# aniketntnu/WordDiffusion

Hardware: AMD Instinct MI355X
Metric: denoised 64x256 word images/sec (1000-step DDPM), whole job (higher is better)
Workload: dtype bf16x3; 1 GPU; BASELINE configs[1]: batch 64 per GPU of 64x256 crops = [64,4,8,32] latents, 1000-step DDPM (999 executed steps), base unet.py UNetModel (320 ch, mult (1,1), 4 heads, 339 writers), random-init synthetic weights; variant=base, batch_per_gpu=64, noise_steps=1000, executed_steps_per_image=999, precision=split-bf16 MFMA x3, fp32 accumulate (<=1e-4 of the fp32 reference), output_finite=True

## Files before the change

worddiffusion_amd/csrc/wd_ff.hip:

```cpp
#include "wd_gemm_epi.h"

namespace {

constexpr int FNT = 512;
constexpr int FBM = 64;
constexpr int FC = 320;
constexpr int FCH = 128;
constexpr int FRING = 6;
constexpr int F_MAX_INNER = 2048;
constexpr int FGRP = 30;
constexpr uint32_t F_OOB = 0x80000000u;

typedef __attribute__((ext_vector_type(4))) unsigned f_u32x4;

__device__ __forceinline__ int f_lds_off(int row, int ch) { return row * 128 + ((ch ^ ((row >> 1) & 7)) << 4); }

template <int NPASS, bool PROJ, bool FRONT>
__global__ void __launch_bounds__(FNT, 1) wd_ff_kernel(const wd_ff_args a) {
#if defined(__HIP_DEVICE_COMPILE__)
    static_assert(!FRONT || (NPASS == 3 && PROJ), "the transformer front needs split-bf16 operands and the proj_out tail");
    constexpr int NPL = (NPASS == 1) ? 1 : 2;
    constexpr int SLAB = 2 * FBM * 128;
    constexpr int A_BYTES = 5 * SLAB;
    constexpr int H_BYTES = 2 * SLAB;
    extern __shared__ __attribute__((aligned(16))) char smem[];
    char* s_a = smem;
    char* s_h = smem + A_BYTES;
    float* s_b1 = reinterpret_cast<float*>(smem + A_BYTES + 2 * H_BYTES);

    const int m0 = blockIdx.x * FBM;
    const int tid = threadIdx.x;
    const int lane = tid & 63;
    const int wave = __builtin_amdgcn_readfirstlane(tid >> 6);
    const int kh = wave >> 2, cg = wave & 3;
    const int l15 = lane & 15, lq = lane >> 4;
    const int nchunk = a.inner / FCH;

    auto make_srd = [](const wd_bf16* p) {
        return __builtin_amdgcn_make_buffer_rsrc(const_cast<wd_bf16*>(p), 0, 0x7FFFFFF0, 0x00020000);
    };
    const __amdgpu_buffer_rsrc_t srd1_hi = make_srd(a.w1_hi), srd1_lo = make_srd(a.w1_lo ? a.w1_lo : a.w1_hi);
    const __amdgpu_buffer_rsrc_t srd2_hi = make_srd(a.w2_hi), srd2_lo = make_srd(a.w2_lo ? a.w2_lo : a.w2_hi);
    const __amdgpu_buffer_rsrc_t srd3_hi = make_srd(PROJ ? a.w3_hi : a.w2_hi), srd3_lo = make_srd(PROJ ? (a.w3_lo ? a.w3_lo : a.w3_hi) : a.w2_hi);
    const uint32_t lane16 = lane * 16;
    const int nct1 = (2 * a.inner) >> 4;

    bf16x8 ring[FRING][NPL];
    auto issue = [&](const int slot, const int g, const int j) {
        const bool live = j < nchunk;
        const uint32_t vo = live ? lane16 : F_OOB;
        if (PROJ && g < FRING) {
            const uint32_t so3 = (uint32_t)(((2 * (g / 5) + kh) * (FC / 16) + 5 * cg + g % 5) * 1024);
            const uint32_t so1 = (uint32_t)(((g >> 1) * nct1 + 2 * (j * 8 + wave) + (g & 1)) * 1024);
            const uint32_t so = live ? so1 : so3;
#pragma unroll
            for (int p = 0; p < NPL; ++p) {
                const __amdgpu_buffer_rsrc_t srd = live ? (p ? srd1_lo : srd1_hi) : (p ? srd3_lo : srd3_hi);
                ring[slot][p] = __builtin_bit_cast(bf16x8, __builtin_amdgcn_raw_buffer_load_b128(srd, lane16, so, 0));
            }
        } else if (g < 20) {
            const uint32_t so = (uint32_t)(((g >> 1) * nct1 + 2 * (j * 8 + wave) + (g & 1)) * 1024);
#pragma unroll
            for (int p = 0; p < NPL; ++p)
                ring[slot][p] = __builtin_bit_cast(bf16x8, __builtin_amdgcn_raw_buffer_load_b128(p ? srd1_lo : srd1_hi, vo, live ? so : 0u, 0));
        } else {
            const int q = (g - 20) / 5, t = (g - 20) % 5;
            const uint32_t so = (uint32_t)(((4 * j + 2 * kh + q) * (FC / 16) + 5 * cg + t) * 1024);
#pragma unroll
            for (int p = 0; p < NPL; ++p)
                ring[slot][p] = __builtin_bit_cast(bf16x8, __builtin_amdgcn_raw_buffer_load_b128(p ? srd2_lo : srd2_hi, vo, live ? so : 0u, 0));
        }
    };
    f32x4 acc2[4][5];
    bf16x8 xa[4][NPL];
    auto read_frags = [&](const char* slab_base, const int half) {
        const int ch = half * 4 + lq;
#pragma unroll
        for (int i = 0; i < 4; ++i) {
            const int ao = f_lds_off(i * 16 + l15, ch);
#pragma unroll
            for (int p = 0; p < NPL; ++p) xa[i][p] = *reinterpret_cast<const bf16x8*>(slab_base + p * (FBM * 128) + ao);
        }
    };
    auto mfma12 = [&](f32x4 (&acc)[4], const bf16x8 (&w)[NPL]) {
#pragma unroll
        for (int i = 0; i < 4; ++i) {
            if (NPL == 2) {
                acc[i] = __builtin_amdgcn_mfma_f32_16x16x32_bf16(xa[i][NPL - 1], w[0], acc[i], 0, 0, 0);
                acc[i] = __builtin_amdgcn_mfma_f32_16x16x32_bf16(xa[i][0], w[NPL - 1], acc[i], 0, 0, 0);
            }
            acc[i] = __builtin_amdgcn_mfma_f32_16x16x32_bf16(xa[i][0], w[0], acc[i], 0, 0, 0);
        }
    };
    constexpr int LDE = FC + 4;
    float* ep = reinterpret_cast<float*>(smem);
    auto ksum_to_image = [&]() {
        for (int hh = 0; hh < 2; ++hh) {
            if (kh == hh) {
#pragma unroll
                for (int i = 0; i < 4; ++i)
#pragma unroll
                    for (int t = 0; t < 5; ++t)
#pragma unroll
                        for (int r = 0; r < 4; ++r) {
                            float* pe = ep + (i * 16 + 4 * lq + r) * LDE + cg * 80 + t * 16 + l15;
                            *pe = (hh == 0) ? acc2[i][t][r] : *pe + acc2[i][t][r];
                        }
            }
            __syncthreads();
        }
    };

    if constexpr (FRONT) {
        constexpr int SP = 65, PP = 72, KS32 = FC / 32;
        const int b = m0 / a.hw;
        const int HJ = a.heads * a.L;
        char* fr = s_h + 4096;
        float* s_aff = reinterpret_cast<float*>(fr);
        float* sS = reinterpret_cast<float*>(fr);
        wd_bf16* sP = reinterpret_cast<wd_bf16*>(fr + FBM * SP * 4);
        {
            const int ngp = FC / a.gn_pcpg, ratio = a.gn_cpg / a.gn_pcpg;
            for (int c = tid; c < FC; c += FNT) {
                const int g = c / a.gn_cpg;
                double su = 0.0, sq = 0.0;
                for (int k = 0; k < ratio; ++k)
                    for (int ck = 0; ck < a.gn_nchunk; ++ck) {
                        const double* pp = a.gn_part + (((long)b * a.gn_nchunk + ck) * ngp + g * ratio + k) * 2;
                        su += pp[0];
                        sq += pp[1];
                    }
                const double n = (double)a.hw * a.gn_cpg;
                const double mu = su / n;
                double var = sq / n - mu * mu;
                if (var < 0.0) var = 0.0;
                const float rstd = (float)(1.0 / sqrt(var + (double)a.gn_eps));
                const float sc = rstd * a.gn_gamma[c];
                s_aff[2 * c] = sc;
                s_aff[2 * c + 1] = a.gn_beta[c] - (float)mu * sc;
            }
            for (int e = tid; e < FBM * PP; e += FNT) reinterpret_cast<uint32_t*>(sP)[e] = 0u;
        }
        const int arow = tid >> 3, ach = tid & 7;
        float4 xv[5][2];
        {
            const float* xrow = a.x_in + (long)(m0 + arow) * a.x_in_ld + ach * 8;
#pragma unroll
            for (int sl = 0; sl < 5; ++sl) {
                xv[sl][0] = *reinterpret_cast<const float4*>(xrow + sl * 64);
                xv[sl][1] = *reinterpret_cast<const float4*>(xrow + sl * 64 + 4);
            }
        }
        const __amdgpu_buffer_rsrc_t srdp_hi = make_srd(a.pi_hi), srdp_lo = make_srd(a.pi_lo);
        auto issue_pi = [&](const int slot, const int g) {
            const uint32_t so = (uint32_t)(((2 * (g / 5) + kh) * (FC / 16) + 5 * cg + g % 5) * 1024);
#pragma unroll
            for (int p = 0; p < NPL; ++p)
                ring[slot][p] = __builtin_bit_cast(bf16x8, __builtin_amdgcn_raw_buffer_load_b128(p ? srdp_lo : srdp_hi, lane16, so, 0));
        };
#pragma unroll
        for (int g = 0; g < FRING; ++g) issue_pi(g, g);
        __syncthreads();
#pragma unroll
        for (int sl = 0; sl < 5; ++sl) {
            const float4* tab = reinterpret_cast<const float4*>(s_aff + 2 * (sl * 64 + ach * 8));
            const float4 t0 = tab[0], t1 = tab[1], t2 = tab[2], t3 = tab[3];
            const float4 x0 = xv[sl][0], x1 = xv[sl][1];
            float4 y0, y1;
            y0.x = x0.x * t0.x + t0.y; y0.y = x0.y * t0.z + t0.w; y0.z = x0.z * t1.x + t1.y; y0.w = x0.w * t1.z + t1.w;
            y1.x = x1.x * t2.x + t2.y; y1.y = x1.y * t2.z + t2.w; y1.z = x1.z * t3.x + t3.y; y1.w = x1.w * t3.z + t3.w;
            uint2 h0, l0, h1, l1;
            wd_split4(y0, h0, l0);
            wd_split4(y1, h1, l1);
            char* dst = s_a + sl * SLAB + f_lds_off(arow, ach);
            *reinterpret_cast<f_u32x4*>(dst) = f_u32x4{h0.x, h0.y, h1.x, h1.y};
            *reinterpret_cast<f_u32x4*>(dst + FBM * 128) = f_u32x4{l0.x, l0.y, l1.x, l1.y};
        }
        __syncthreads();
#pragma unroll
        for (int i = 0; i < 4; ++i)
#pragma unroll
            for (int t = 0; t < 5; ++t)
#pragma unroll
                for (int r = 0; r < 4; ++r) acc2[i][t][r] = 0.0f;
#pragma unroll
        for (int g = 0; g < 25; ++g) {
            const int q = g / 5, t = g % 5;
            if (t == 0) read_frags(s_a + q * SLAB, kh);
            {
                f32x4 col[4] = {acc2[0][t], acc2[1][t], acc2[2][t], acc2[3][t]};
                mfma12(col, ring[g % FRING]);
#pragma unroll
                for (int i = 0; i < 4; ++i) acc2[i][t] = col[i];
            }
            if (g + FRING < 25) issue_pi(g % FRING, g + FRING);
            __builtin_amdgcn_sched_barrier(0);
        }
        __syncthreads();
        ksum_to_image();
        float4 xr[2][5];
#pragma unroll
        for (int pp = 0; pp < 2; ++pp)
#pragma unroll
            for (int i = 0; i < 5; ++i) {
                const int n = (l15 + 16 * i) * 4, row = wave * 8 + pp * 4 + lq;
                const float4 v = *reinterpret_cast<const float4*>(ep + row * LDE + n);
                const float4 bx = *reinterpret_cast<const float4*>(a.pi_b + n);
                xr[pp][i] = make_float4(v.x + bx.x, v.y + bx.y, v.z + bx.z, v.w + bx.w);
            }
        __syncthreads();
        auto ln_rows = [&](const float* gamma, const float* beta) {
#pragma unroll
            for (int pp = 0; pp < 2; ++pp) {
                const int row = wave * 8 + pp * 4 + lq;
                float s = 0.f;
#pragma unroll
                for (int i = 0; i < 5; ++i) s += (xr[pp][i].x + xr[pp][i].y) + (xr[pp][i].z + xr[pp][i].w);
                const float mean = wd_row16_sum(s) / (float)FC;
                float q = 0.f;
#pragma unroll
                for (int i = 0; i < 5; ++i) {
                    const float a0 = xr[pp][i].x - mean, a1 = xr[pp][i].y - mean, a2 = xr[pp][i].z - mean, a3 = xr[pp][i].w - mean;
                    q += (a0 * a0 + a1 * a1) + (a2 * a2 + a3 * a3);
                }
                const float rstd = 1.0f / sqrtf(wd_row16_sum(q) / (float)FC + a.ln_eps);
#pragma unroll
                for (int i = 0; i < 5; ++i) {
                    const int n = (l15 + 16 * i) * 4;
                    const float4 ga = *reinterpret_cast<const float4*>(gamma + n);
                    const float4 be = *reinterpret_cast<const float4*>(beta + n);
                    const float4 x = xr[pp][i];
                    float4 o;
                    o.x = (x.x - mean) * rstd * ga.x + be.x; o.y = (x.y - mean) * rstd * ga.y + be.y;
                    o.z = (x.z - mean) * rstd * ga.z + be.z; o.w = (x.w - mean) * rstd * ga.w + be.w;
                    uint2 hi, lo;
                    wd_split4(o, hi, lo);
                    char* d = s_a + (n >> 6) * SLAB + f_lds_off(row, (n & 63) >> 3) + (n & 7) * 2;
                    *reinterpret_cast<uint2*>(d) = hi;
                    *reinterpret_cast<uint2*>(d + FBM * 128) = lo;
                }
            }
        };
        const int ht = wave & 3, rp = wave >> 2;
        const long pq = 64L * FC;
#pragma unroll
        for (int ps = 0; ps < 2; ++ps) {
            const wd_bf16* mq = ps == 0 ? a.mq_a : a.mq_b;
            const wd_bf16* mot = ps == 0 ? a.mot_a : a.mot_b;
            const float* xb = ps == 0 ? a.xb_a : a.xb_b;
            ln_rows(a.ln2_gamma, a.ln2_beta);
            __builtin_amdgcn_sched_barrier(0);
            bf16x8 bh[KS32], bl[KS32];
            {
                const __amdgpu_buffer_rsrc_t rq = __builtin_amdgcn_make_buffer_rsrc(const_cast<wd_bf16*>(mq + (long)b * 2 * pq), 0,
                                                                                    (int)(2 * pq * 2), 0x00020000);
                const uint32_t vo = ht * 16 + l15 < HJ ? lane16 : F_OOB;
#pragma unroll
                for (int ks = 0; ks < KS32; ++ks) {
                    bh[ks] = __builtin_bit_cast(bf16x8, __builtin_amdgcn_raw_buffer_load_b128(rq, vo, (uint32_t)((ht * KS32 + ks) << 10), 0));
                    bl[ks] = __builtin_bit_cast(bf16x8, __builtin_amdgcn_raw_buffer_load_b128(rq, vo, (uint32_t)(((ht * KS32 + ks) << 10) + pq * 2), 0));
                }
            }
            __syncthreads();
            if (ht * 16 < HJ) {
                f32x4 a_lh[2], a_hl[2], a_hh[2];
#pragma unroll
                for (int ri = 0; ri < 2; ++ri)
#pragma unroll
                    for (int r = 0; r < 4; ++r) a_lh[ri][r] = a_hl[ri][r] = a_hh[ri][r] = 0.f;
#pragma unroll
                for (int ks = 0; ks < KS32; ++ks)
#pragma unroll
                    for (int ri = 0; ri < 2; ++ri) {
                        const char* ap = s_a + (ks >> 1) * SLAB + f_lds_off((2 * rp + ri) * 16 + l15, (ks & 1) * 4 + lq);
                        const bf16x8 ah = *reinterpret_cast<const bf16x8*>(ap);
                        const bf16x8 al = *reinterpret_cast<const bf16x8*>(ap + FBM * 128);
                        a_lh[ri] = __builtin_amdgcn_mfma_f32_16x16x32_bf16(al, bh[ks], a_lh[ri], 0, 0, 0);
                        a_hl[ri] = __builtin_amdgcn_mfma_f32_16x16x32_bf16(ah, bl[ks], a_hl[ri], 0, 0, 0);
                        a_hh[ri] = __builtin_amdgcn_mfma_f32_16x16x32_bf16(ah, bh[ks], a_hh[ri], 0, 0, 0);
                    }
#pragma unroll
                for (int ri = 0; ri < 2; ++ri)
#pragma unroll
                    for (int r = 0; r < 4; ++r)
                        sS[((2 * rp + ri) * 16 + 4 * lq + r) * SP + ht * 16 + l15] = (a_lh[ri][r] + a_hl[ri][r]) + a_hh[ri][r];
            }
            __builtin_amdgcn_sched_barrier(0);
            bf16x8 mh[2][5], ml[2][5];
            {
                const __amdgpu_buffer_rsrc_t rm = __builtin_amdgcn_make_buffer_rsrc(const_cast<wd_bf16*>(mot + (long)b * 2 * pq), 0,
                                                                                    (int)(2 * pq * 2), 0x00020000);
#pragma unroll
                for (int ks = 0; ks < 2; ++ks) {
                    const uint32_t vo = ks * 32 + lq * 8 < HJ ? lane16 : F_OOB;
#pragma unroll
                    for (int t = 0; t < 5; ++t) {
                        const uint32_t so = (uint32_t)((((5 * cg + t) * 2 + ks) << 10));
                        mh[ks][t] = __builtin_bit_cast(bf16x8, __builtin_amdgcn_raw_buffer_load_b128(rm, vo, so, 0));
                        ml[ks][t] = __builtin_bit_cast(bf16x8, __builtin_amdgcn_raw_buffer_load_b128(rm, vo, so + (uint32_t)(pq * 2), 0));
                    }
                }
            }
            __syncthreads();
            for (int idx = tid; idx < FBM * a.heads; idx += FNT) {
                const int t = idx / a.heads, h = idx - t * a.heads;
                const float* pr = sS + t * SP + h * a.L;
                wd_bf16* ph = sP + t * PP + h * a.L;
                float mx = -3.4e38f;
                for (int j = 0; j < a.L; ++j) mx = fmaxf(mx, pr[j]);
                float sum = 0.f;
                for (int j = 0; j < a.L; ++j) sum += __expf(pr[j] - mx);
                const float inv = __fdividef(1.f, sum);
                for (int j = 0; j < a.L; ++j) {
                    uint32_t hi, lo;
                    wd_split1(__expf(pr[j] - mx) * inv, hi, lo);
                    ph[j] = (wd_bf16)hi;
                    ph[FBM * PP + j] = (wd_bf16)lo;
                }
            }
            __syncthreads();
            {
                f32x4 o[2][5];
#pragma unroll
                for (int ri = 0; ri < 2; ++ri)
#pragma unroll
                    for (int t = 0; t < 5; ++t)
#pragma unroll
                        for (int r = 0; r < 4; ++r) o[ri][t][r] = 0.f;
#pragma unroll
                for (int ks = 0; ks < 2; ++ks)
#pragma unroll
                    for (int ri = 0; ri < 2; ++ri) {
                        const wd_bf16* ap = sP + ((2 * rp + ri) * 16 + l15) * PP + lq * 8 + ks * 32;
                        const bf16x8 ah = *reinterpret_cast<const bf16x8*>(ap);
                        const bf16x8 al = *reinterpret_cast<const bf16x8*>(ap + FBM * PP);
#pragma unroll
                        for (int t = 0; t < 5; ++t) o[ri][t] = __builtin_amdgcn_mfma_f32_16x16x32_bf16(al, mh[ks][t], o[ri][t], 0, 0, 0);
#pragma unroll
                        for (int t = 0; t < 5; ++t) o[ri][t] = __builtin_amdgcn_mfma_f32_16x16x32_bf16(ah, ml[ks][t], o[ri][t], 0, 0, 0);
#pragma unroll
                        for (int t = 0; t < 5; ++t) o[ri][t] = __builtin_amdgcn_mfma_f32_16x16x32_bf16(ah, mh[ks][t], o[ri][t], 0, 0, 0);
                    }
#pragma unroll
                for (int ri = 0; ri < 2; ++ri)
#pragma unroll
                    for (int t = 0; t < 5; ++t)
#pragma unroll
                        for (int r = 0; r < 4; ++r) ep[((2 * rp + ri) * 16 + 4 * lq + r) * LDE + (5 * cg + t) * 16 + l15] = o[ri][t][r];
            }
            __syncthreads();
#pragma unroll
            for (int pp = 0; pp < 2; ++pp)
#pragma unroll
                for (int i = 0; i < 5; ++i) {
                    const int n = (l15 + 16 * i) * 4, row = wave * 8 + pp * 4 + lq;
                    const float4 bi = *reinterpret_cast<const float4*>(xb + n);
                    const float4 at = *reinterpret_cast<const float4*>(ep + row * LDE + n);
                    const float4 x = xr[pp][i];
                    xr[pp][i] = make_float4(at.x + bi.x + x.x, at.y + bi.y + x.y, at.z + bi.z + x.z, at.w + bi.w + x.w);
                }
            __syncthreads();
        }
#pragma unroll
        for (int pp = 0; pp < 2; ++pp)
#pragma unroll
            for (int i = 0; i < 5; ++i)
                *reinterpret_cast<float4*>(a.tok2 + (long)(m0 + wave * 8 + pp * 4 + lq) * FC + (l15 + 16 * i) * 4) = xr[pp][i];
        ln_rows(a.ln3_gamma, a.ln3_beta);
        for (int i = tid; i < 2 * a.inner; i += FNT) s_b1[i] = a.b1 ? a.b1[i] : 0.0f;
        __builtin_amdgcn_sched_barrier(0);
#pragma unroll
        for (int g = 0; g < FRING; ++g) issue(g, g, 0);
    } else {
#pragma unroll
    for (int g = 0; g < FRING; ++g) issue(g, g, 0);

    {
        const __amdgpu_buffer_rsrc_t sx_hi = make_srd(a.x_hi), sx_lo = make_srd(a.x_lo ? a.x_lo : a.x_hi);
        const int arow = tid >> 3, ach = tid & 7;
        const uint32_t vo = (m0 + arow < a.m) ? (uint32_t)(m0 + arow) * (uint32_t)(a.x_ld * 2) + (uint32_t)(ach * 16) : F_OOB;
        f_u32x4 v[5][NPL];
#pragma unroll
        for (int sl = 0; sl < 5; ++sl)
#pragma unroll
            for (int p = 0; p < NPL; ++p) v[sl][p] = __builtin_amdgcn_raw_buffer_load_b128(p ? sx_lo : sx_hi, vo, sl * 128, 0);
        const int dst = f_lds_off(arow, ach);
#pragma unroll
        for (int sl = 0; sl < 5; ++sl)
#pragma unroll
            for (int p = 0; p < NPL; ++p) *reinterpret_cast<f_u32x4*>(s_a + sl * SLAB + p * (FBM * 128) + dst) = v[sl][p];
        for (int i = tid; i < 2 * a.inner; i += FNT) s_b1[i] = a.b1 ? a.b1[i] : 0.0f;
    }
    }
    __syncthreads();

#pragma unroll
    for (int i = 0; i < 4; ++i)
#pragma unroll
        for (int t = 0; t < 5; ++t)
#pragma unroll
            for (int r = 0; r < 4; ++r) acc2[i][t][r] = 0.0f;

    for (int j = 0; j < nchunk; ++j) {
        char* hbuf = s_h + (j & 1) * H_BYTES;
        f32x4 ax[4], ag[4];
#pragma unroll
        for (int i = 0; i < 4; ++i)
#pragma unroll
            for (int r = 0; r < 4; ++r) {
                ax[i][r] = 0.0f;
                ag[i][r] = 0.0f;
            }
#pragma unroll
        for (int g = 0; g < 20; ++g) {
            if ((g & 1) == 0) read_frags(s_a + (g >> 2) * SLAB, (g >> 1) & 1);
            if (g & 1) mfma12(ag, ring[g % FRING]);
            else mfma12(ax, ring[g % FRING]);
            if (g + FRING < FGRP) issue(g % FRING, g + FRING, j);
            else issue(g % FRING, g + FRING - FGRP, j + 1);
            __builtin_amdgcn_sched_barrier(0);
        }
        {
            const int hcol = (j * 8 + wave) * 32 + l15;
            const float bx = s_b1[hcol], bg = s_b1[hcol + 16];
            const int slab = wave >> 2, ch = (wave & 3) * 2 + (l15 >> 3), e = (l15 & 7) * 2;
#pragma unroll
            for (int i = 0; i < 4; ++i)
#pragma unroll
                for (int r = 0; r < 4; ++r) {
                    const float h = (ax[i][r] + bx) * wd_gelu_erf(ag[i][r] + bg);
                    uint32_t hb, lb;
                    wd_split1(h, hb, lb);
                    char* p = hbuf + slab * SLAB + f_lds_off(i * 16 + lq * 4 + r, ch) + e;
                    *reinterpret_cast<unsigned short*>(p) = (unsigned short)hb;
                    if (NPL == 2) *reinterpret_cast<unsigned short*>(p + FBM * 128) = (unsigned short)lb;
                }
        }
        __syncthreads();
#pragma unroll
        for (int g = 20; g < FGRP; ++g) {
            const int q = (g - 20) / 5, t = (g - 20) % 5;
            if (t == 0) read_frags(hbuf + kh * SLAB, q);
            {
                f32x4 col[4] = {acc2[0][t], acc2[1][t], acc2[2][t], acc2[3][t]};
                mfma12(col, ring[g % FRING]);
#pragma unroll
                for (int i = 0; i < 4; ++i) acc2[i][t] = col[i];
            }
            if (g + FRING < FGRP) issue(g % FRING, g + FRING, j);
            else issue(g % FRING, g + FRING - FGRP, j + 1);
            __builtin_amdgcn_sched_barrier(0);
        }
    }

    __syncthreads();
    ksum_to_image();
    wd_gemm_args e = {};
    e.m = a.m;
    e.n = FC;
    e.hw_out = a.hw_out > 0 ? a.hw_out : 1;
    e.act = WD_ACT_NONE;
    e.out_f32 = a.out_f32;
    e.out_ld = a.out_ld;
    e.out_hi = a.out_hi;
    e.out_lo = a.out_lo;
    e.out_pl_ld = a.out_pl_ld;
    e.ksplit = 1;
    e.stat_part = a.stat_part;
    e.stat_cpg = a.stat_cpg;
    if constexpr (!PROJ) {
        e.bias = a.b2;
        e.resid = a.resid;
        e.resid_ld = a.resid_ld;
        wd_epilogue_from_image<FBM, FC, FNT>(e, ep, m0, 0, tid);
    } else {
        constexpr int ROWB = LDE * 4;
        const float* resid = FRONT ? a.tok2 : a.resid;
        const int resid_ld = FRONT ? FC : a.resid_ld;
        if (FRONT) asm volatile("s_waitcnt vmcnt(0)" ::: "memory");
        {
            float4 v[10];
#pragma unroll
            for (int it = 0; it < 10; ++it) {
                const int idx = it * 64 + lane, row = wave * 8 + idx / 80, c = (idx % 80) * 4;
                const int m = m0 + row;
                float4 x = *reinterpret_cast<const float4*>(ep + row * LDE + c);
                if (a.b2) {
                    const float4 q = *reinterpret_cast<const float4*>(a.b2 + c);
                    x.x += q.x; x.y += q.y; x.z += q.z; x.w += q.w;
                }
                if (resid && m < a.m) {
                    const float4 q = *reinterpret_cast<const float4*>(resid + (long)m * resid_ld + c);
                    x.x += q.x; x.y += q.y; x.z += q.z; x.w += q.w;
                }
                v[it] = x;
            }
            asm volatile("s_waitcnt lgkmcnt(0)" ::: "memory");
            __builtin_amdgcn_sched_barrier(0);
#pragma unroll
            for (int it = 0; it < 10; ++it) {
                const int idx = it * 64 + lane, row = wave * 8 + idx / 80, c = (idx % 80) * 4;
                uint2 hh, ll;
                wd_split4(v[it], hh, ll);
                char* rowp = reinterpret_cast<char*>(ep) + row * ROWB;
                *reinterpret_cast<uint2*>(rowp + c * 2) = hh;
                if (NPL == 2) *reinterpret_cast<uint2*>(rowp + 640 + c * 2) = ll;
            }
        }
        __syncthreads();
#pragma unroll
        for (int i = 0; i < 4; ++i)
#pragma unroll
            for (int t = 0; t < 5; ++t)
#pragma unroll
                for (int r = 0; r < 4; ++r) acc2[i][t][r] = 0.0f;
#pragma unroll
        for (int g = 0; g < 25; ++g) {
            const int q = g / 5, t = g % 5;
            if (t == 0) {
                const int ks = 2 * q + kh;
#pragma unroll
                for (int i = 0; i < 4; ++i) {
                    const char* rp = reinterpret_cast<const char*>(ep) + (i * 16 + l15) * ROWB + (ks * 4 + lq) * 16;
#pragma unroll
                    for (int p = 0; p < NPL; ++p) xa[i][p] = *reinterpret_cast<const bf16x8*>(rp + p * 640);
// ... 85 lines not shown
```

worddiffusion_amd/csrc/wd_norm.hip:

```cpp
#include "wd_common.h"

namespace {

constexpr int GN_TOK = 32;

__global__ void gn_stats_kernel(const float* __restrict__ x, int ld, int hw, int c, int cpg, int nchunk,
                                double* __restrict__ part) {
    extern __shared__ __attribute__((aligned(16))) char smem[];
    float* s_sum = reinterpret_cast<float*>(smem);
    float* s_sq = s_sum + 2 * c;
    const int b = blockIdx.y, j = blockIdx.x;
    const int cx = threadIdx.x * 4;
    const int t0 = j * GN_TOK, t1 = min(hw, t0 + GN_TOK);
    if (cx < c) {
        float4 s = make_float4(0, 0, 0, 0), q = make_float4(0, 0, 0, 0);
        const float* base = x + ((long)b * hw) * ld + cx;
        for (int t = t0 + threadIdx.y; t < t1; t += 2) {
            const float4 v = *reinterpret_cast<const float4*>(base + (long)t * ld);
            s.x += v.x; s.y += v.y; s.z += v.z; s.w += v.w;
            q.x += v.x * v.x; q.y += v.y * v.y; q.z += v.z * v.z; q.w += v.w * v.w;
        }
        *reinterpret_cast<float4*>(s_sum + threadIdx.y * c + cx) = s;
        *reinterpret_cast<float4*>(s_sq + threadIdx.y * c + cx) = q;
    }
// ... 51 lines not shown
    }
    __syncthreads();
    const int c4 = c >> 2;
    const int t0 = blockIdx.x * AP_TOK, nt = min(AP_TOK, hw - t0);
    if (c4 <= 256) {
        const int rpp = 256 / c4;
        const int tl = threadIdx.x / c4, cx = (threadIdx.x - tl * c4) * 4;
        if (tl >= rpp) return;
        float sc[4], sh[4];
#pragma unroll
        for (int j = 0; j < 4; ++j) {
            const int g = (cx + j) / cpg;
            sc[j] = s_rstd[g] * gamma[c_off + cx + j];
            sh[j] = beta[c_off + cx + j] - s_mean[g] * sc[j];
        }
        for (int t = tl; t < nt; t += rpp) {
            const long row = (long)b * hw + t0 + t;
            const long srow = sr.perm ? (long)b * hw + sr.perm[t0 + t] : row;
            const float4 v = *reinterpret_cast<const float4*>(x + srow * ld + cx);
            float4 y = make_float4(v.x * sc[0] + sh[0], v.y * sc[1] + sh[1], v.z * sc[2] + sh[2], v.w * sc[3] + sh[3]);
            if (silu) {
                y.x = wd_silu(y.x); y.y = wd_silu(y.y); y.z = wd_silu(y.z); y.w = wd_silu(y.w);
            }
            uint2 h, l;
            wd_split4(y, h, l);
            const long o = row * out_ld + c_off + cx;
            *reinterpret_cast<uint2*>(out_hi + o) = h;
            if (out_lo) *reinterpret_cast<uint2*>(out_lo + o) = l;
            if (raw_hi) {
                wd_split4(v, h, l);
                *reinterpret_cast<uint2*>(raw_hi + o) = h;
                if (raw_lo) *reinterpret_cast<uint2*>(raw_lo + o) = l;
            }
        }
        return;
    }
    const int total = nt * c4;
    for (int i = threadIdx.x; i < total; i += blockDim.x) {
        const int t = i / c4, cx = (i - t * c4) * 4;
        const long row = (long)b * hw + t0 + t;
        const long srow = sr.perm ? (long)b * hw + sr.perm[t0 + t] : row;
        const float4 v = *reinterpret_cast<const float4*>(x + srow * ld + cx);
        float4 y;
        {
            const int g = cx / cpg, g1 = (cx + 1) / cpg, g2 = (cx + 2) / cpg, g3 = (cx + 3) / cpg;
            const float4 ga = *reinterpret_cast<const float4*>(gamma + c_off + cx);
            const float4 be = *reinterpret_cast<const float4*>(beta + c_off + cx);
            const float s0 = s_rstd[g] * ga.x, s1 = s_rstd[g1] * ga.y, s2 = s_rstd[g2] * ga.z, s3 = s_rstd[g3] * ga.w;
            y.x = v.x * s0 + (be.x - s_mean[g] * s0);
            y.y = v.y * s1 + (be.y - s_mean[g1] * s1);
            y.z = v.z * s2 + (be.z - s_mean[g2] * s2);
            y.w = v.w * s3 + (be.w - s_mean[g3] * s3);
        }
        if (silu) {
            y.x = wd_silu(y.x); y.y = wd_silu(y.y); y.z = wd_silu(y.z); y.w = wd_silu(y.w);
        }
        uint2 h, l;
        wd_split4(y, h, l);
        const long o = row * out_ld + c_off + cx;
        *reinterpret_cast<uint2*>(out_hi + o) = h;
        if (out_lo) *reinterpret_cast<uint2*>(out_lo + o) = l;
        if (raw_hi) {
            wd_split4(v, h, l);
            *reinterpret_cast<uint2*>(raw_hi + o) = h;
            if (raw_lo) *reinterpret_cast<uint2*>(raw_lo + o) = l;
        }
    }
}

constexpr int LN_MAX4 = 8;
__global__ void layernorm_kernel(const float* __restrict__ x, int ld, int rows, int c, const float* __restrict__ gamma,
                                 const float* __restrict__ beta, float eps, wd_bf16* __restrict__ out_hi,
                                 wd_bf16* __restrict__ out_lo, int out_ld) {
    const int lane = threadIdx.x & 63;
    const int row = blockIdx.x * (blockDim.x >> 6) + (threadIdx.x >> 6);
    if (row >= rows) return;
    const int c4 = c >> 2;
    float4 v[LN_MAX4];
    float s = 0.f;
#pragma unroll
    for (int i = 0; i < LN_MAX4; ++i) {
        const int f = lane + 64 * i;
        if (f < c4) {
            v[i] = *reinterpret_cast<const float4*>(x + (long)row * ld + f * 4);
            s += (v[i].x + v[i].y) + (v[i].z + v[i].w);
        }
    }
    const float mean = wd_wave_sum(s) / (float)c;
    float q = 0.f;
#pragma unroll
    for (int i = 0; i < LN_MAX4; ++i) {
        const int f = lane + 64 * i;
        if (f < c4) {
            const float a = v[i].x - mean, b = v[i].y - mean, cc = v[i].z - mean, d = v[i].w - mean;
            q += (a * a + b * b) + (cc * cc + d * d);
        }
    }
    const float rstd = 1.0f / sqrtf(wd_wave_sum(q) / (float)c + eps);
#pragma unroll
    for (int i = 0; i < LN_MAX4; ++i) {
        const int f = lane + 64 * i;
        if (f < c4) {
            const float4 ga = *reinterpret_cast<const float4*>(gamma + f * 4);
            const float4 be = *reinterpret_cast<const float4*>(beta + f * 4);
            float4 y;
            y.x = (v[i].x - mean) * rstd * ga.x + be.x;
            y.y = (v[i].y - mean) * rstd * ga.y + be.y;
            y.z = (v[i].z - mean) * rstd * ga.z + be.z;
            y.w = (v[i].w - mean) * rstd * ga.w + be.w;
            uint2 h, l;
            wd_split4(y, h, l);
            const long o = (long)row * out_ld + f * 4;
            *reinterpret_cast<uint2*>(out_hi + o) = h;
            if (out_lo) *reinterpret_cast<uint2*>(out_lo + o) = l;
        }
    }
}

__global__ void split_kernel(const float* __restrict__ x, int ld, int rows, int c, int silu,
                             wd_bf16* __restrict__ out_hi, wd_bf16* __restrict__ out_lo, int out_ld) {
    const int c4 = c >> 2;
    const long total = (long)rows * c4;
    for (long i = (long)blockIdx.x * blockDim.x + threadIdx.x; i < total; i += (long)gridDim.x * blockDim.x) {
        const long r = i / c4;
        const int cx = (int)(i - r * c4) * 4;
        float4 v = *reinterpret_cast<const float4*>(x + r * ld + cx);
        if (silu) {
            v.x = wd_silu(v.x); v.y = wd_silu(v.y); v.z = wd_silu(v.z); v.w = wd_silu(v.w);
        }
        uint2 h, l;
        wd_split4(v, h, l);
        *reinterpret_cast<uint2*>(out_hi + r * out_ld + cx) = h;
        if (out_lo) *reinterpret_cast<uint2*>(out_lo + r * out_ld + cx) = l;
    }
}

constexpr int GC_CH = 64;
constexpr int GC_PITCH = GC_CH + 4;
template <int PXL>
__global__ void __launch_bounds__(256) gn_conv_few_kernel(const float* __restrict__ x, int ld, int H, int W, int c, int cpg, int nchunk,
                                                         int part_cpg, const double* __restrict__ part,
                                                         const float* __restrict__ gamma, const float* __restrict__ beta, float eps,
                                                         int silu, const float* __restrict__ w, const float* __restrict__ bias, int oc,
                                                         float* __restrict__ out) {
    constexpr int CG = 256 / PXL, CPT = GC_CH / CG;
    constexpr int NLD = 3 * PXL * (GC_CH / 4) / 256;
    extern __shared__ __attribute__((aligned(16))) char smem[];
    float* s_w = reinterpret_cast<float*>(smem);
    float* s_t = s_w + 9 * GC_CH * 4;
    __shared__ float s_mean[32], s_rstd[32];
    const int b = blockIdx.x, y = blockIdx.y, tid = threadIdx.x;
    const int hw = H * W, ng = c / cpg;
    float4 pv[NLD];
    auto request = [&](int c0) {
#pragma unroll
        for (int k = 0; k < NLD; ++k) {
            const int i = tid + 256 * k;
            const int r = i / (PXL * (GC_CH / 4)), rem = i - r * (PXL * (GC_CH / 4));
            const int px = rem / (GC_CH / 4), c4 = rem - px * (GC_CH / 4);
            const int yy = y + r - 1;
            pv[k] = (yy >= 0 && yy < H && px < W)
                        ? *reinterpret_cast<const float4*>(x + ((long)b * hw + (long)yy * W + px) * ld + c0 + c4 * 4)
                        : make_float4(0.f, 0.f, 0.f, 0.f);
        }
    };
    request(0);
    if (tid < ng) {
        const int ratio = cpg / part_cpg, ngs = c / part_cpg;
        double ds = 0.0, dq = 0.0;
        for (int j = 0; j < nchunk; ++j) {
            const double* p = part + (((long)b * nchunk + j) * ngs + tid * ratio) * 2;
            for (int k = 0; k < ratio; ++k) {
                ds += p[2 * k];
                dq += p[2 * k + 1];
            }
        }
        const double n = (double)hw * cpg;
        const double mean = ds / n;
        double var = dq / n - mean * mean;
        if (var < 0.0) var = 0.0;
        s_mean[tid] = (float)mean;
        s_rstd[tid] = (float)(1.0 / sqrt(var + (double)eps));
    }
    for (int i = tid; i < 3 * 2 * (GC_CH / 4); i += 256) {
        const int r = i / (2 * (GC_CH / 4)), rem = i - r * (2 * (GC_CH / 4));
        const int side = rem / (GC_CH / 4), c4 = rem - side * (GC_CH / 4);
        *reinterpret_cast<float4*>(s_t + ((long)r * (W + 2) + (side ? W + 1 : 0)) * GC_PITCH + c4 * 4) = make_float4(0.f, 0.f, 0.f, 0.f);
    }
    for (int i = tid; i < 9 * GC_CH; i += 256) *reinterpret_cast<float4*>(s_w + (long)i * 4) = make_float4(0.f, 0.f, 0.f, 0.f);
    __syncthreads();
    const int pl = tid % PXL, cg = tid / PXL;
    float4 acc = make_float4(0.f, 0.f, 0.f, 0.f);
    for (int c0 = 0; c0 < c; c0 += GC_CH) {
        for (int i = tid; i < oc * GC_CH * 9; i += 256) {
            const int o = i / (GC_CH * 9), rem = i - o * (GC_CH * 9);
            s_w[rem * 4 + o] = w[((long)o * c + c0) * 9 + rem];
        }
        float sc[4], sh[4];
        {
            const int ch = c0 + (tid & (GC_CH / 4 - 1)) * 4;
#pragma unroll
            for (int j = 0; j < 4; ++j) {
                const int g = (ch + j) / cpg;
                sc[j] = s_rstd[g] * gamma[ch + j];
                sh[j] = beta[ch + j] - s_mean[g] * sc[j];
            }
        }
#pragma unroll
        for (int k = 0; k < NLD; ++k) {
            const int i = tid + 256 * k;
            const int r = i / (PXL * (GC_CH / 4)), rem = i - r * (PXL * (GC_CH / 4));
            const int px = rem / (GC_CH / 4), c4 = rem - px * (GC_CH / 4);
            const int yy = y + r - 1;
            if (px >= W) continue;
            float4 o = make_float4(0.f, 0.f, 0.f, 0.f);
            if (yy >= 0 && yy < H) {
                const float4 v = pv[k];
                o = make_float4(v.x * sc[0] + sh[0], v.y * sc[1] + sh[1], v.z * sc[2] + sh[2], v.w * sc[3] + sh[3]);
                if (silu) {
                    o.x = wd_silu(o.x); o.y = wd_silu(o.y); o.z = wd_silu(o.z); o.w = wd_silu(o.w);
                }
            }
            *reinterpret_cast<float4*>(s_t + ((long)r * (W + 2) + px + 1) * GC_PITCH + c4 * 4) = o;
        }
        if (c0 + GC_CH < c) request(c0 + GC_CH);
        __syncthreads();
        if (pl < W) {
#pragma unroll
            for (int dy = 0; dy < 3; ++dy)
#pragma unroll
                for (int dx = 0; dx < 3; ++dx) {
                    const float* at = s_t + ((long)dy * (W + 2) + pl + dx) * GC_PITCH + cg * CPT;
                    const float* wt = s_w + ((long)(cg * CPT) * 9 + dy * 3 + dx) * 4;
#pragma unroll
                    for (int k = 0; k < CPT / 4; ++k) {
                        const float4 a = *reinterpret_cast<const float4*>(at + 4 * k);
                        const float4 w0 = *reinterpret_cast<const float4*>(wt + (4 * k + 0) * 36);
                        const float4 w1 = *reinterpret_cast<const float4*>(wt + (4 * k + 1) * 36);
                        const float4 w2 = *reinterpret_cast<const float4*>(wt + (4 * k + 2) * 36);
                        const float4 w3 = *reinterpret_cast<const float4*>(wt + (4 * k + 3) * 36);
                        acc.x += a.x * w0.x; acc.y += a.x * w0.y; acc.z += a.x * w0.z; acc.w += a.x * w0.w;
                        acc.x += a.y * w1.x; acc.y += a.y * w1.y; acc.z += a.y * w1.z; acc.w += a.y * w1.w;
                        acc.x += a.z * w2.x; acc.y += a.z * w2.y; acc.z += a.z * w2.z; acc.w += a.z * w2.w;
                        acc.x += a.w * w3.x; acc.y += a.w * w3.y; acc.z += a.w * w3.z; acc.w += a.w * w3.w;
                    }
                }
        }
        __syncthreads();
    }
    float* s_red = s_t;
    *reinterpret_cast<float4*>(s_red + ((long)cg * PXL + pl) * 4) = acc;
    __syncthreads();
    for (int i = tid; i < W * oc; i += 256) {
        const int o = i / W, px = i - o * W;
        float v = bias ? bias[o] : 0.f;
        for (int g = 0; g < CG; ++g) v += s_red[((long)g * PXL + px) * 4 + o];
        out[(((long)b * oc + o) * H + y) * W + px] = v;
    }
}

__global__ void __launch_bounds__(256) gn_fold_chunks_kernel(const double* __restrict__ part, int nchunk, int ng2,
                                                            double* __restrict__ out) {
    __shared__ double red[4][64];
    const int col = threadIdx.x & 63, lane = threadIdx.x >> 6;
    const long b = blockIdx.x;
    double acc = 0.0;
    if (col < ng2)
        for (int j = lane; j < nchunk; j += 4) acc += part[(b * nchunk + j) * ng2 + col];
    red[lane][col] = acc;
    __syncthreads();
    if (lane == 0 && col < ng2) out[b * ng2 + col] = (red[0][col] + red[1][col]) + (red[2][col] + red[3][col]);
}

}

extern "C" int wd_gn_nchunk(int hw) { return (hw + GN_TOK - 1) / GN_TOK; }

extern "C" int wd_gn_fold_chunks(const double* part, int batch, int nchunk, int ngroups, double* out, void* stream) {
    if (!part || !out || batch <= 0 || nchunk <= 0 || ngroups <= 0 || ngroups > 32) return WD_EINVAL;
    hipStream_t st = reinterpret_cast<hipStream_t>(stream);
    WdLaunchScope scope(WD_CLS_GNSTATS, st);
    hipLaunchKernelGGL(gn_fold_chunks_kernel, dim3(batch), dim3(256), 0, st, part, nchunk, 2 * ngroups, out);
    return wd_check_launch();
}

extern "C" int wd_gn_stats(const float* x, int ld, int batch, int hw, int c, int cpg, double* part, void* stream) {
    if (!x || !part || batch <= 0 || hw <= 0 || c <= 0 || cpg <= 0) return WD_EINVAL;
    if (c % 4 || ld % 4 || c % cpg || c / cpg > 256 || c > 4096) return WD_EINVAL;
    hipStream_t st = reinterpret_cast<hipStream_t>(stream);
    const int nchunk = wd_gn_nchunk(hw);
    const int bx = 64 * ((c / 4 + 63) / 64);
    if (bx * 2 > 1024) return WD_EINVAL;
    WdLaunchScope scope(WD_CLS_GNSTATS, st);
    hipLaunchKernelGGL(gn_stats_kernel, dim3(nchunk, batch), dim3(bx, 2), 4 * c * sizeof(float), st, x, ld, hw, c, cpg,
                       nchunk, part);
    return wd_check_launch();
}

extern "C" int wd_gn_apply(const float* x, int ld, int batch, int hw, int c, int cpg, const double* part, int nchunk,
                           int part_cpg, const float* gamma, const float* beta, float eps, int silu, wd_bf16* out_hi,
                           wd_bf16* out_lo, int out_ld, int c_off, wd_bf16* raw_hi, wd_bf16* raw_lo, void* stream) {
    if (!x || !part || !gamma || !beta || !out_hi || batch <= 0 || hw <= 0 || nchunk <= 0 || part_cpg <= 0) return WD_EINVAL;
    if (c % 4 || ld % 4 || out_ld % 4 || c_off % 4 || c % cpg || c / cpg > 32 || cpg % part_cpg) return WD_EINVAL;
    hipStream_t st = reinterpret_cast<hipStream_t>(stream);
    WdLaunchScope scope(WD_CLS_GNAPPLY, st);
    const GnSrc s0 = {x, part, ld, c, nchunk, part_cpg, c_off, nullptr};
    hipLaunchKernelGGL(gn_apply_kernel, dim3((hw + AP_TOK - 1) / AP_TOK, batch, 1), dim3(256), 0, st, s0, s0, hw, cpg, gamma, beta, eps,
                       silu, out_hi, out_lo, out_ld, raw_hi, raw_lo);
    return wd_check_launch();
}

extern "C" int wd_gn_apply2(const float* xa, int lda, int ca, const double* part_a, int nchunk_a, int part_cpg_a, int c_off_a,
                            const float* xb, int ldb, int cb, const double* part_b, int nchunk_b, int part_cpg_b, int c_off_b,
                            int batch, int hw, int cpg, const float* gamma, const float* beta, float eps, int silu,
                            wd_bf16* out_hi, wd_bf16* out_lo, int out_ld, wd_bf16* raw_hi, wd_bf16* raw_lo, const int32_t* perm_a,
                            void* stream) {
    if (!xa || !xb || !part_a || !part_b || !gamma || !beta || !out_hi || batch <= 0 || hw <= 0 || nchunk_a <= 0 || nchunk_b <= 0 ||
        part_cpg_a <= 0 || part_cpg_b <= 0)
        return WD_EINVAL;
    if (ca % 4 || cb % 4 || lda % 4 || ldb % 4 || out_ld % 4 || c_off_a % 4 || c_off_b % 4 || ca % cpg || cb % cpg ||
        ca / cpg > 32 || cb / cpg > 32 || cpg % part_cpg_a || cpg % part_cpg_b)
        return WD_EINVAL;
    hipStream_t st = reinterpret_cast<hipStream_t>(stream);
    WdLaunchScope scope(WD_CLS_GNAPPLY, st);
    const GnSrc s0 = {xa, part_a, lda, ca, nchunk_a, part_cpg_a, c_off_a, perm_a}, s1 = {xb, part_b, ldb, cb, nchunk_b, part_cpg_b, c_off_b, nullptr};
    hipLaunchKernelGGL(gn_apply_kernel, dim3((hw + AP_TOK - 1) / AP_TOK, batch, 2), dim3(256), 0, st, s0, s1, hw, cpg, gamma, beta, eps,
                       silu, out_hi, out_lo, out_ld, raw_hi, raw_lo);
    return wd_check_launch();
}

static int gn_conv_tile_floats(int w) { return 3 * (w + 2) * GC_PITCH > 1024 ? 3 * (w + 2) * GC_PITCH : 1024; }

extern "C" int wd_gn_conv3x3_few_supported(int c, int w, int oc) {
    return c > 0 && c % GC_CH == 0 && w > 0 && w <= 64 && oc >= 1 && oc <= 4 &&
           (size_t)(9 * GC_CH * 4 + gn_conv_tile_floats(w)) * sizeof(float) <= 64 * 1024;
}

extern "C" int wd_gn_conv3x3_few(const float* x, int ld, int batch, int h, int w, int c, int cpg, const double* part, int nchunk,
                                 int part_cpg, const float* gamma, const float* beta, float eps, int silu, const float* weight,
                                 const float* bias, int oc, float* out, void* stream) {
    if (!x || !part || !gamma || !beta || !weight || !out || batch <= 0 || h <= 0 || nchunk <= 0 || part_cpg <= 0) return WD_EINVAL;
    if (!wd_gn_conv3x3_few_supported(c, w, oc) || ld % 4 || cpg <= 0 || c % cpg || c / cpg > 32 || cpg % part_cpg) return WD_EINVAL;
    hipStream_t st = reinterpret_cast<hipStream_t>(stream);
    const size_t smem = (size_t)(9 * GC_CH * 4 + gn_conv_tile_floats(w)) * sizeof(float);
    WdLaunchScope scope(WD_CLS_OTHER, st);
    if (w <= 32)
        hipLaunchKernelGGL(gn_conv_few_kernel<32>, dim3(batch, h), dim3(256), smem, st, x, ld, h, w, c, cpg, nchunk, part_cpg, part,
                           gamma, beta, eps, silu, weight, bias, oc, out);
    else
        hipLaunchKernelGGL(gn_conv_few_kernel<64>, dim3(batch, h), dim3(256), smem, st, x, ld, h, w, c, cpg, nchunk, part_cpg, part,
                           gamma, beta, eps, silu, weight, bias, oc, out);
    return wd_check_launch();
}

extern "C" int wd_layernorm(const float* x, int ld, int rows, int c, const float* gamma, const float* beta, float eps,
                            wd_bf16* out_hi, wd_bf16* out_lo, int out_ld, void* stream) {
    if (!x || !gamma || !beta || !out_hi || rows <= 0 || c <= 0) return WD_EINVAL;
    if (c % 4 || ld % 4 || out_ld % 4 || c > 64 * 4 * LN_MAX4) return WD_EINVAL;
// ... 18 lines not shown
```

Baseline: 34.93 images/s.

## Prefetch norm partials, per-channel vectors and weights early to hide global load latency

In the transformer front kernel, the GroupNorm partial sums, gamma/beta, bias and LayerNorm vectors are now issued as register loads at kernel start and staged into LDS. The cross-attention mq operand loads are hoisted so the second pass's loads are issued during the first pass. The proj_in/FF weight ring prefetch is also issued before the final LayerNorm. In the GroupNorm+conv kernel, conv weights and gamma/beta are loaded into registers together with the activation prefetch, replacing serialized global reads inside the channel loop. The aim is to overlap dependent global-memory latency with other work, at the cost of higher register pressure and extra LDS use.

```diff
diff --git a/worddiffusion_amd/csrc/wd_ff.hip b/worddiffusion_amd/csrc/wd_ff.hip
--- a/worddiffusion_amd/csrc/wd_ff.hip
+++ b/worddiffusion_amd/csrc/wd_ff.hip
@@ -10,6 +10,8 @@
 constexpr int F_MAX_INNER = 2048;
 constexpr int FGRP = 30;
 constexpr uint32_t F_OOB = 0x80000000u;
+constexpr int F_NVEC = 7;
+constexpr int F_VEC_OFF = 40960;
 
 typedef __attribute__((ext_vector_type(4))) unsigned f_u32x4;
 
@@ -119,47 +121,85 @@
         float* s_aff = reinterpret_cast<float*>(fr);
         float* sS = reinterpret_cast<float*>(fr);
         wd_bf16* sP = reinterpret_cast<wd_bf16*>(fr + FBM * SP * 4);
+        float* s_vec = reinterpret_cast<float*>(s_h + F_VEC_OFF);
+        static_assert(4096 + FBM * SP * 4 + 2 * FBM * PP * 2 <= F_VEC_OFF && F_VEC_OFF + F_NVEC * FC * 4 <= H_BYTES * 2, "front LDS");
+        constexpr int NPART = 8;
+        const int ngp = FC / a.gn_pcpg, ratio = a.gn_cpg / a.gn_pcpg, npart = ratio * a.gn_nchunk;
+        const int c = tid < FC ? tid : 0;
+        const int grp = c / a.gn_cpg;
+        auto part_at = [&](const int mi) {
+            const int k = mi / a.gn_nchunk, ck = mi - k * a.gn_nchunk;
+            return a.gn_part + (((long)b * a.gn_nchunk + ck) * ngp + grp * ratio + k) * 2;
+        };
+        double2 pr[NPART];
+#pragma unroll
+        for (int mi = 0; mi < NPART; ++mi) pr[mi] = *reinterpret_cast<const double2*>(part_at(mi < npart ? mi : 0));
+        const float gga = a.gn_gamma[c], gbe = a.gn_beta[c];
+        const int arow = tid >> 3, ach = tid & 7;
+        float4 xv[5][2];
         {
-            const int ngp = FC / a.gn_pcpg, ratio = a.gn_cpg / a.gn_pcpg;
-            for (int c = tid; c < FC; c += FNT) {
-                const int g = c / a.gn_cpg;
+            const float* xrow = a.x_in + (long)(m0 + arow) * a.x_in_ld + ach * 8;
+#pragma unroll
+            for (int sl = 0; sl < 5; ++sl) {
+                xv[sl][0] = *reinterpret_cast<const float4*>(xrow + sl * 64);
+                xv[sl][1] = *reinterpret_cast<const float4*>(xrow + sl * 64 + 4);
+            }
+        }
+        const __amdgpu_buffer_rsrc_t srdp_hi = make_srd(a.pi_hi), srdp_lo = make_srd(a.pi_lo);
+        auto issue_pi = [&](const int slot, const int g) {
+            const uint32_t so = (uint32_t)(((2 * (g / 5) + kh) * (FC / 16) + 5 * cg + g % 5) * 1024);
+#pragma unroll
+            for (int p = 0; p < NPL; ++p)
+                ring[slot][p] = __builtin_bit_cast(bf16x8, __builtin_amdgcn_raw_buffer_load_b128(p ? srdp_lo : srdp_hi, lane16, so, 0));
+        };
+#pragma unroll
+        for (int g = 0; g < FRING; ++g) issue_pi(g, g);
+        constexpr int NB1 = 2 * F_MAX_INNER / 4 / FNT;
+        const int vq = tid < FC / 4 ? tid : 0;
+        float4 vv[F_NVEC], b1v[NB1];
+        int b1q[NB1];
+        {
+            const float* vsrc[F_NVEC] = {a.pi_b, a.ln2_gamma, a.ln2_beta, a.xb_a, a.xb_b, a.ln3_gamma, a.ln3_beta};
+#pragma unroll
+            for (int v = 0; v < F_NVEC; ++v) vv[v] = *reinterpret_cast<const float4*>(vsrc[v] + 4 * vq);
+            const float* b1src = a.b1 ? a.b1 : a.pi_b;
+#pragma unroll
+            for (int k = 0; k < NB1; ++k) {
+                b1q[k] = a.b1 && tid + FNT * k < a.inner / 2 ? tid + FNT * k : 0;
+                const float* pb = b1src + 4 * b1q[k];
+                b1v[k] = make_float4(pb[0], pb[1], pb[2], pb[3]);
+            }
+        }
+        {
+#pragma unroll
+            for (int v = 0; v < F_NVEC; ++v) reinterpret_cast<float4*>(s_vec + v * FC)[vq] = vv[v];
+#pragma unroll
+            for (int k = 0; k < NB1; ++k)
+                reinterpret_cast<float4*>(s_b1)[b1q[k]] = a.b1 ? b1v[k] : make_float4(0.f, 0.f, 0.f, 0.f);
+            if (tid < FC) {
                 double su = 0.0, sq = 0.0;
-                for (int k = 0; k < ratio; ++k)
-                    for (int ck = 0; ck < a.gn_nchunk; ++ck) {
-                        const double* pp = a.gn_part + (((long)b * a.gn_nchunk + ck) * ngp + g * ratio + k) * 2;
-                        su += pp[0];
-                        sq += pp[1];
+#pragma unroll
+                for (int mi = 0; mi < NPART; ++mi)
+                    if (mi < npart) {
+                        su += pr[mi].x;
+                        sq += pr[mi].y;
                     }
+                for (int mi = NPART; mi < npart; ++mi) {
+                    const double* pp = part_at(mi);
+                    su += pp[0];
+                    sq += pp[1];
+                }
                 const double n = (double)a.hw * a.gn_cpg;
                 const double mu = su / n;
                 double var = sq / n - mu * mu;
                 if (var < 0.0) var = 0.0;
                 const float rstd = (float)(1.0 / sqrt(var + (double)a.gn_eps));
-                const float sc = rstd * a.gn_gamma[c];
+                const float sc = rstd * gga;
                 s_aff[2 * c] = sc;
-                s_aff[2 * c + 1] = a.gn_beta[c] - (float)mu * sc;
+                s_aff[2 * c + 1] = gbe - (float)mu * sc;
             }
             for (int e = tid; e < FBM * PP; e += FNT) reinterpret_cast<uint32_t*>(sP)[e] = 0u;
         }
-        const int arow = tid >> 3, ach = tid & 7;
-        float4 xv[5][2];
-        {
-            const float* xrow = a.x_in + (long)(m0 + arow) * a.x_in_ld + ach * 8;
-#pragma unroll
-            for (int sl = 0; sl < 5; ++sl) {
-                xv[sl][0] = *reinterpret_cast<const float4*>(xrow + sl * 64);
-                xv[sl][1] = *reinterpret_cast<const float4*>(xrow + sl * 64 + 4);
-            }
-        }
-        const __amdgpu_buffer_rsrc_t srdp_hi = make_srd(a.pi_hi), srdp_lo = make_srd(a.pi_lo);
-        auto issue_pi = [&](const int slot, const int g) {
-            const uint32_t so = (uint32_t)(((2 * (g / 5) + kh) * (FC / 16) + 5 * cg + g % 5) * 1024);
-#pragma unroll
-            for (int p = 0; p < NPL; ++p)
-                ring[slot][p] = __builtin_bit_cast(bf16x8, __builtin_amdgcn_raw_buffer_load_b128(p ? srdp_lo : srdp_hi, lane16, so, 0));
-        };
-#pragma unroll
-        for (int g = 0; g < FRING; ++g) issue_pi(g, g);
         __syncthreads();
 #pragma unroll
         for (int sl = 0; sl < 5; ++sl) {
@@ -197,6 +237,20 @@
             __builtin_amdgcn_sched_barrier(0);
         }
         __syncthreads();
+        const int ht = wave & 3, rp = wave >> 2;
+        const long pq = 64L * FC;
+        bf16x8 bh[KS32], bl[KS32];
+        auto request_mq = [&](const wd_bf16* mq) {
+            const __amdgpu_buffer_rsrc_t rq = __builtin_amdgcn_make_buffer_rsrc(const_cast<wd_bf16*>(mq + (long)b * 2 * pq), 0,
+                                                                                (int)(2 * pq * 2), 0x00020000);
+            const uint32_t vo = ht * 16 + l15 < HJ ? lane16 : F_OOB;
+#pragma unroll
+            for (int ks = 0; ks < KS32; ++ks) {
+                bh[ks] = __builtin_bit_cast(bf16x8, __builtin_amdgcn_raw_buffer_load_b128(rq, vo, (uint32_t)((ht * KS32 + ks) << 10), 0));
+                bl[ks] = __builtin_bit_cast(bf16x8, __builtin_amdgcn_raw_buffer_load_b128(rq, vo, (uint32_t)(((ht * KS32 + ks) << 10) + pq * 2), 0));
+            }
+        };
+        request_mq(a.mq_a);
         ksum_to_image();
         float4 xr[2][5];
 #pragma unroll
@@ -205,7 +259,7 @@
             for (int i = 0; i < 5; ++i) {
                 const int n = (l15 + 16 * i) * 4, row = wave * 8 + pp * 4 + lq;
                 const float4 v = *reinterpret_cast<const float4*>(ep + row * LDE + n);
-                const float4 bx = *reinterpret_cast<const float4*>(a.pi_b + n);
+                const float4 bx = *reinterpret_cast<const float4*>(s_vec + n);
                 xr[pp][i] = make_float4(v.x + bx.x, v.y + bx.y, v.z + bx.z, v.w + bx.w);
             }
         __syncthreads();
@@ -241,26 +295,12 @@
                 }
             }
         };
-        const int ht = wave & 3, rp = wave >> 2;
-        const long pq = 64L * FC;
 #pragma unroll
         for (int ps = 0; ps < 2; ++ps) {
-            const wd_bf16* mq = ps == 0 ? a.mq_a : a.mq_b;
             const wd_bf16* mot = ps == 0 ? a.mot_a : a.mot_b;
-            const float* xb = ps == 0 ? a.xb_a : a.xb_b;
-            ln_rows(a.ln2_gamma, a.ln2_beta);
+            const float* xb = s_vec + (ps == 0 ? 3 : 4) * FC;
+            ln_rows(s_vec + FC, s_vec + 2 * FC);
             __builtin_amdgcn_sched_barrier(0);
-            bf16x8 bh[KS32], bl[KS32];
-            {
-                const __amdgpu_buffer_rsrc_t rq = __builtin_amdgcn_make_buffer_rsrc(const_cast<wd_bf16*>(mq + (long)b * 2 * pq), 0,
-                                                                                    (int)(2 * pq * 2), 0x00020000);
-                const uint32_t vo = ht * 16 + l15 < HJ ? lane16 : F_OOB;
-#pragma unroll
-                for (int ks = 0; ks < KS32; ++ks) {
-                    bh[ks] = __builtin_bit_cast(bf16x8, __builtin_amdgcn_raw_buffer_load_b128(rq, vo, (uint32_t)((ht * KS32 + ks) << 10), 0));
-                    bl[ks] = __builtin_bit_cast(bf16x8, __builtin_amdgcn_raw_buffer_load_b128(rq, vo, (uint32_t)(((ht * KS32 + ks) << 10) + pq * 2), 0));
-                }
-            }
             __syncthreads();
             if (ht * 16 < HJ) {
                 f32x4 a_lh[2], a_hl[2], a_hh[2];
@@ -348,6 +388,7 @@
 #pragma unroll
                         for (int r = 0; r < 4; ++r) ep[((2 * rp + ri) * 16 + 4 * lq + r) * LDE + (5 * cg + t) * 16 + l15] = o[ri][t][r];
             }
+            if (ps == 0) request_mq(a.mq_b);
             __syncthreads();
 #pragma unroll
             for (int pp = 0; pp < 2; ++pp)
@@ -362,15 +403,14 @@
             __syncthreads();
         }
 #pragma unroll
+        for (int g = 0; g < FRING; ++g) issue(g, g, 0);
+        __builtin_amdgcn_sched_barrier(0);
+#pragma unroll
         for (int pp = 0; pp < 2; ++pp)
 #pragma unroll
             for (int i = 0; i < 5; ++i)
                 *reinterpret_cast<float4*>(a.tok2 + (long)(m0 + wave * 8 + pp * 4 + lq) * FC + (l15 + 16 * i) * 4) = xr[pp][i];
-        ln_rows(a.ln3_gamma, a.ln3_beta);
-        for (int i = tid; i < 2 * a.inner; i += FNT) s_b1[i] = a.b1 ? a.b1[i] : 0.0f;
-        __builtin_amdgcn_sched_barrier(0);
-#pragma unroll
-        for (int g = 0; g < FRING; ++g) issue(g, g, 0);
+        ln_rows(s_vec + 5 * FC, s_vec + 6 * FC);
     } else {
 #pragma unroll
     for (int g = 0; g < FRING; ++g) issue(g, g, 0);
diff --git a/worddiffusion_amd/csrc/wd_norm.hip b/worddiffusion_amd/csrc/wd_norm.hip
--- a/worddiffusion_amd/csrc/wd_norm.hip
+++ b/worddiffusion_amd/csrc/wd_norm.hip
@@ -227,6 +227,9 @@
     const int b = blockIdx.x, y = blockIdx.y, tid = threadIdx.x;
     const int hw = H * W, ng = c / cpg;
     float4 pv[NLD];
+    constexpr int NW = 9 * GC_CH * 4 / 256;
+    float wv[NW];
+    float4 gv, bv;
     auto request = [&](int c0) {
 #pragma unroll
         for (int k = 0; k < NLD; ++k) {
@@ -238,17 +241,40 @@
                         ? *reinterpret_cast<const float4*>(x + ((long)b * hw + (long)yy * W + px) * ld + c0 + c4 * 4)
                         : make_float4(0.f, 0.f, 0.f, 0.f);
         }
+#pragma unroll
+        for (int k = 0; k < NW; ++k) {
+            const int i = tid + 256 * k;
+            const int o = i / (GC_CH * 9), rem = i - o * (GC_CH * 9);
+            const float v = w[((long)(o < oc ? o : 0) * c + c0) * 9 + rem];
+            wv[k] = o < oc ? v : 0.f;
+        }
+        const int ch = c0 + (tid & (GC_CH / 4 - 1)) * 4;
+        gv = make_float4(gamma[ch], gamma[ch + 1], gamma[ch + 2], gamma[ch + 3]);
+        bv = make_float4(beta[ch], beta[ch + 1], beta[ch + 2], beta[ch + 3]);
     };
+    constexpr int NPART = 8;
+    const int ratio = cpg / part_cpg, ngs = c / part_cpg, npart = nchunk * ratio;
+    const int pg = tid < ng ? tid : 0;
+    auto part_at = [&](int mi) {
+        const int j = mi / ratio, k = mi - j * ratio;
+        return part + (((long)b * nchunk + j) * ngs + pg * ratio) * 2 + 2 * k;
+    };
+    double2 pr[NPART];
+#pragma unroll
+    for (int mi = 0; mi < NPART; ++mi) pr[mi] = *reinterpret_cast<const double2*>(part_at(mi < npart ? mi : 0));
     request(0);
     if (tid < ng) {
-        const int ratio = cpg / part_cpg, ngs = c / part_cpg;
         double ds = 0.0, dq = 0.0;
-        for (int j = 0; j < nchunk; ++j) {
-            const double* p = part + (((long)b * nchunk + j) * ngs + tid * ratio) * 2;
-            for (int k = 0; k < ratio; ++k) {
-                ds += p[2 * k];
-                dq += p[2 * k + 1];
-            }
+#pragma unroll
+        for (int mi = 0; mi < NPART; ++mi)
+            if (mi < npart) {
+                ds += pr[mi].x;
+                dq += pr[mi].y;
+            }
+        for (int mi = NPART; mi < npart; ++mi) {
+            const double* p = part_at(mi);
+            ds += p[0];
+            dq += p[1];
         }
         const double n = (double)hw * cpg;
         const double mean = ds / n;
@@ -262,23 +288,25 @@
         const int side = rem / (GC_CH / 4), c4 = rem - side * (GC_CH / 4);
         *reinterpret_cast<float4*>(s_t + ((long)r * (W + 2) + (side ? W + 1 : 0)) * GC_PITCH + c4 * 4) = make_float4(0.f, 0.f, 0.f, 0.f);
     }
-    for (int i = tid; i < 9 * GC_CH; i += 256) *reinterpret_cast<float4*>(s_w + (long)i * 4) = make_float4(0.f, 0.f, 0.f, 0.f);
     __syncthreads();
     const int pl = tid % PXL, cg = tid / PXL;
     float4 acc = make_float4(0.f, 0.f, 0.f, 0.f);
     for (int c0 = 0; c0 < c; c0 += GC_CH) {
-        for (int i = tid; i < oc * GC_CH * 9; i += 256) {
+#pragma unroll
+        for (int k = 0; k < NW; ++k) {
+            const int i = tid + 256 * k;
             const int o = i / (GC_CH * 9), rem = i - o * (GC_CH * 9);
-            s_w[rem * 4 + o] = w[((long)o * c + c0) * 9 + rem];
+            s_w[rem * 4 + o] = wv[k];
         }
         float sc[4], sh[4];
         {
             const int ch = c0 + (tid & (GC_CH / 4 - 1)) * 4;
+            const float ga[4] = {gv.x, gv.y, gv.z, gv.w}, be[4] = {bv.x, bv.y, bv.z, bv.w};
 #pragma unroll
             for (int j = 0; j < 4; ++j) {
                 const int g = (ch + j) / cpg;
-                sc[j] = s_rstd[g] * gamma[ch + j];
-                sh[j] = beta[ch + j] - s_mean[g] * sc[j];
+                sc[j] = s_rstd[g] * ga[j];
+                sh[j] = be[j] - s_mean[g] * sc[j];
             }
         }
 #pragma unroll
```

Result: faster. 35.42 images/s (median of 6 runs) (+1.4%).
